# ShengkaiWu/IoU-aware-single-stage-object-detector

Hardware: AMD Instinct MI355X
Metric: images/sec at 1333x800, IoU-aware RetinaNet R-50-FPN (higher is better)
Workload: dtype fp32; 1 GPU; IoU-aware RetinaNet R-50-FPN fp32, batch 8 per GPU, 3x800x1344 (1333x800 padded to /32), random-init weights, whole inference path incl. NMS, device-to-host copy and bbox2result (the reference's simple_test: per-class arrays on the host; batch i's host part runs under batch i+1's device part, the last one inside the timed region); global_batch=8, parallelism=dp1, dets_per_image=100

## Files before the change

### include/iouaware.h

```cpp
#ifndef IOUAWARE_H
#define IOUAWARE_H

#include <stddef.h>
#include <stdint.h>

#ifdef __cplusplus
extern "C" {
#endif

#define IA_MAX_LEVELS 8
#define IA_MAX_ANCHORS 16
#define IA_MAX_NMS_PRE 4096
#define IA_MAX_CANDIDATES 8192
#define IA_MAX_PER_IMG 1024

#define IA_F32 0
#define IA_BF16 1
#define IA_F16 2
#define IA_F64 3

#define IA_LAYOUT_NCHW 0
#define IA_LAYOUT_NHWC 1

#define IA_CLS_SIGMOID 0
// ... 124 lines not shown
    int32_t dst_channels, dst_offset;
    float *dst[IA_MAX_LEVELS];
} ia_wino_seg;
int ia_wino_tiles(const ia_wino_geom *g, int32_t *tiles);
int ia_wino_input_transform(const ia_wino_geom *g, const float *const *x, int channels, int groups,
                            const float *pre_scale, const float *pre_shift, int pre_relu, float *V,
                            void *stream);
int ia_wino_output_transform(const ia_wino_geom *g, const float *M, int channels, int groups,
                             const float *bias, int relu, int nseg, const ia_wino_seg *segs,
                             void *stream);
int ia_wino_mid_transform(const ia_wino_geom *g, const float *M, int channels, int groups_m,
                          const float *bias, int relu, float *V, int groups_v, void *stream);
int ia_wino_in_gemm(const ia_wino_geom *g, const float *const *x, int channels, const float *pre_scale,
                    const float *pre_shift, int pre_relu, const float *u_packed, float *M, void *stream);

int ia_wino_grad_output_transform(const ia_wino_geom *g, const float *const *dy, int channels,
                                  float *dM, void *stream);

#define IA_COLSUM_MAX_STRIPS 512
size_t ia_relu_bwd_bias_grad_workspace_bytes(int64_t rows, int n);
int ia_wino_weight_transform(const float *w, int n_in, int n_out, int64_t stride_in,
                             int64_t stride_out, int64_t stride_ky, int64_t stride_kx, int flip,
                             const double *G, float *U, void *stream);
int ia_wino_weight_grad(const float *dU, int n_in, int n_out, const double *G, float *dW,
                        int64_t stride_in, int64_t stride_out, int64_t stride_ky, int64_t stride_kx,
                        void *stream);
int ia_bn_fold_fwd(const float *w, const float *gamma, const float *beta, const float *mean,
                   const float *inv_std, int cout, int K, float *w_out, float *b_out, void *stream);
int ia_bn_fold_bwd(const float *dw_folded, const float *db_folded, const float *w, const float *gamma,
                   const float *mean, const float *inv_std, int cout, int K, float *dw,
                   float *dgamma, float *dbeta, void *stream);
int ia_relu_bwd_bias_grad(const float *dy, const float *y, int64_t rows, int n, float *g, float *db,
                          void *workspace, size_t workspace_bytes, void *stream);

int ia_linear_bias_act(const float *A, const float *W, const float *bias, const float *residual,
                       float *D, int64_t rows, int k, int n, int relu, void *workspace,
                       size_t workspace_bytes, void *stream);
int ia_linear_bias_act_bf16(const void *A, const void *W, const float *bias, const void *residual,
                            void *D, int64_t rows, int k, int n, int relu, void *workspace,
                            size_t workspace_bytes, void *stream);
int ia_batched_gemm(const float *A, const float *W, float *D, int batch, int64_t rows, int k, int n,
                    void *workspace, size_t workspace_bytes, void *stream);
int ia_batched_gemm_stream(const float *A, const float *W, float *D, int batch, int64_t rows, int k,
                           int n, void *stream);

size_t ia_im2col3x3_bytes(int B, int H, int W, int C, int stride, int dtype);
int ia_im2col3x3_nhwc(const void *x, void *col, int B, int H, int W, int C, int stride, int dtype,
                      void *stream);
int ia_conv1x1_strided(const void *x, const void *W_kn, const float *bias, const void *residual,
                       void *D, int B, int H, int W, int k, int n, int stride, int relu, int dtype,
                       void *workspace, size_t workspace_bytes, void *stream);
int ia_col2im3x3_nhwc(const void *dcol, void *dx, int B, int H, int W, int C, int stride, int dtype,
                      void *stream);

size_t ia_deform_im2col3x3_bytes(int B, int H, int W, int C, int stride, int pad, int dil);
int ia_deform_im2col3x3_nhwc(const float *x, const float *offset, int64_t offset_pix_stride,
                             const float *mask, int64_t mask_pix_stride, int mask_logits,
                             float *col, int B, int H, int W, int C, int stride, int pad,
                             int dil, int deformable_groups, void *stream);
int ia_deform_col2im3x3_nhwc(const float *dcol, const float *x, const float *offset,
                             int64_t offset_pix_stride, const float *mask,
                             int64_t mask_pix_stride, float *dx, float *d_offset, float *d_mask,
                             int B, int H, int W, int C, int stride, int pad, int dil,
                             int deformable_groups, void *stream);

int ia_gemm_tuning(int mode);

int ia_gemm_table_add(int64_t m, int64_t n, int64_t k, int flags, int batch, int dtype,
                      int solution_index);
int ia_gemm_table_clear(void);
int ia_gemm_table_dump(int64_t *rows7, int capacity);
int ia_gemm_table_stats(int64_t *hits_misses_stale);
int ia_gemm_library_version(void);

int ia_linear_bias_act_wt(const float *A, const float *W_nk, const float *bias,
                          const float *residual, float *D, int64_t rows, int k, int n, int relu,
                          void *workspace, size_t workspace_bytes, void *stream);
int ia_gemm_tn(const float *G, const float *X, float *D, int batch, int64_t rows, int n, int k,
               void *workspace, size_t workspace_bytes, void *stream);


int ia_focal_loss_fwd(const void *cls, int dtype, const int64_t *labels,
                      const float *label_weights, int B, int A, int C, int HW, float gamma,
                      float alpha, double *loss_sum, void *stream);
int ia_focal_loss_bwd(const void *cls, int dtype, const int64_t *labels,
                      const float *label_weights, int B, int A, int C, int HW, float gamma,
                      float alpha, float gscale, const float *gscale_dev, float *grad_cls,
                      void *stream);

int ia_smooth_l1_fwd(const void *pred, int dtype, const float *target, const float *weight,
                     int B, int A, int HW, float beta, double *loss_sum, void *stream);
int ia_smooth_l1_bwd(const void *pred, int dtype, const float *target, const float *weight,
                     int B, int A, int HW, float beta, float gscale, const float *gscale_dev,
                     float *grad_pred, void *stream);

int ia_balanced_l1_fwd(const void *pred, int dtype, const float *target, const float *weight,
                       int B, int A, int HW, float beta, float alpha, float gamma, double *loss_sum,
                       void *stream);
int ia_balanced_l1_bwd(const void *pred, int dtype, const float *target, const float *weight,
                       int B, int A, int HW, float beta, float alpha, float gamma, float gscale,
                       const float *gscale_dev, float *grad_pred, void *stream);

int ia_focal_loss_balanced_fwd(const void *cls, int dtype, const int64_t *labels,
                               const float *label_weights, const float *anchor_iou, int B, int A,
                               int C, int HW, float gamma, float alpha, float eta,
                               double *loss_sums3, void *stream);
// ... 345 lines not shown
```

### iou-aware-single-stage-object-detector_amd/csrc/build.py

```python
import os
import subprocess
import sys

HERE = os.path.dirname(os.path.abspath(__file__))
SOURCES = ['capi.hip', 'decode.hip', 'select.hip', 'nms.hip', 'loss.hip', 'elementwise.hip', 'assign.hip',
           'softnms.hip', 'preproc.hip', 'wino.hip', 'gemm.hip', 'lazynms.hip', 'headloss.hip', 'gconv.hip',
           'trainops.hip', 'bignms.hip', 'conv3x3_bf16.hip', 'conv3x3_bf16_bwd.hip', 'conv1x1_stream.hip', 'im2col.hip', 'nms64.hip', 'stem.hip',
           'groupnorm.hip', 'pointdecode.hip', 'pointloss.hip', 'gconv_bf16.hip', 'gconv_bwd.hip', 'deform.hip']
HEADERS = ['ia_math.hpp', 'ia_block.hpp', 'ia_internal.hpp', 'ia_loss.hpp', 'ia_headloss.hpp', 'ia_rowmax_dev.hpp', 'ia_gather_dev.hpp', 'ia_nms.hpp', 'ia_conv3.hpp', 'ia_wino.hpp', '../../include/iouaware.h']
OUT = os.path.join(HERE, 'libiouaware_hip.so')
FLAGS = ['--offload-arch=gfx950', '-O3', '-std=c++17', '-fPIC', '-ffp-contract=off',
         '-fhip-fp32-correctly-rounded-divide-sqrt', '-fno-gpu-rdc',
         '-Wall', '-Wno-unused-function']


def _hipcc():
    for c in (os.environ.get('HIPCC'), '/opt/rocm/bin/hipcc', 'hipcc'):
        if c and (os.path.isabs(c) and os.path.exists(c) or not os.path.isabs(c)):
            return c
    return 'hipcc'


def needs_build():
    if not os.path.exists(OUT):
        return True
    t = os.path.getmtime(OUT)
    deps = [os.path.join(HERE, f) for f in SOURCES + HEADERS] + [os.path.abspath(__file__)]
    return any(os.path.getmtime(d) > t for d in deps)


def build(force=False, verbose=False):
    if not force and not needs_build():
        return OUT
    objs = []
    procs = []
    for src in SOURCES:
        obj = os.path.join(HERE, src.replace('.hip', '.o'))
        cmd = [_hipcc()] + FLAGS + ['-c', os.path.join(HERE, src), '-o', obj]
        if verbose:
            print(' '.join(cmd))
        procs.append((src, subprocess.Popen(cmd, stdout=subprocess.PIPE, stderr=subprocess.STDOUT)))
        objs.append(obj)
    for src, pr in procs:
        out, _ = pr.communicate()
        if pr.returncode != 0:
            raise RuntimeError('hipcc failed on %s:\n%s' % (src, out.decode()))
        if verbose and out:
            print(out.decode())
    cmd = [_hipcc(), '--offload-arch=gfx950', '-shared', '-fPIC', '-o', OUT] + objs + [
        '-L/opt/rocm/lib', '-lhipblaslt', '-Wl,-rpath,/opt/rocm/lib']
    subprocess.run(cmd, check=True)
    return OUT


if __name__ == '__main__':
    print(build(force='--force' in sys.argv, verbose=True))
```

### iou-aware-single-stage-object-detector_amd/iouaware/_lib.py

```python
import ctypes as C
import os

IA_MAX_LEVELS = 8
IA_MAX_ANCHORS = 16
IA_MAX_NMS_PRE = 4096
IA_MAX_CANDIDATES = 8192
IA_MAX_PER_IMG = 1024
IA_F32, IA_BF16, IA_F16, IA_F64 = 0, 1, 2, 3
IA_LAYOUT_NCHW, IA_LAYOUT_NHWC = 0, 1
IA_CLS_SIGMOID, IA_CLS_SOFTMAX = 0, 1
IA_CLS_SIGMOID_NOIOU, IA_CLS_SOFTMAX_NOIOU = 2, 3
IA_LOSS_SLOTS = 64
IA_MAX_TARGET_BATCH = 16
IA_GN_CHUNK = 256

_CSRC = os.path.join(os.path.dirname(os.path.abspath(__file__)), '..', 'csrc')
SO_PATH = os.path.abspath(os.path.join(_CSRC, 'libiouaware_hip.so'))


class HeadGeom(C.Structure):
    _fields_ = [('num_levels', C.c_int32), ('num_anchors', C.c_int32),
                ('num_classes', C.c_int32), ('nms_pre', C.c_int32),
                ('H', C.c_int32 * IA_MAX_LEVELS), ('W', C.c_int32 * IA_MAX_LEVELS),
                ('stride', C.c_int32 * IA_MAX_LEVELS),
# ... 170 lines not shown
    'ia_focal_loss_balanced_fwd': (_i, [_vp, _i, _vp, _vp, _vp, _i, _i, _i, _i, _f, _f, _f, _vp, _vp]),
    'ia_focal_loss_balanced_bwd': (_i, [_vp, _i, _vp, _vp, _vp, _i, _i, _i, _i, _f, _f, _f, _vp, _f,
                                        _vp, _vp, _vp]),
    'ia_smooth_l1_balanced_fwd': (_i, [_vp, _i, _vp, _vp, _vp, _i, _i, _i, _f, _f, _vp, _vp]),
    'ia_smooth_l1_balanced_bwd': (_i, [_vp, _i, _vp, _vp, _vp, _i, _i, _i, _f, _f, _f, _vp, _vp,
                                       _vp]),
    'ia_iou_bce_fwd': (_i, [_G, _i, _vp, _vp, _i, _vp, _vp, _i, _vp, _vp, _vp]),
    'ia_iou_bce_bwd': (_i, [_G, _i, _vp, _vp, _i, _vp, _vp, _i, _f, _vp, _vp, _vp, _vp]),
    'ia_anchor_targets': (_i, [_G, _vp, _vp, _vp, _i, _i, _vp, _f, _f, _f, _f, _vp, _vp, _vp, _vp,
                               _vp, _vp, _vp]),
    'ia_anchor_targets_ptrs': (_i, [_G, C.POINTER(C.c_void_p), C.POINTER(C.c_void_p),
                                    C.POINTER(C.c_int32), _i, C.POINTER(C.c_int32), _f, _f, _f, _f,
                                    _vp, _vp, _vp, _vp, _vp, _vp, _vp]),
    'ia_head_loss_workspace_bytes': (_sz, [_G, _i]),
    'ia_head_loss_workspace_bytes_cfg': (_sz, [_G, _i, C.POINTER(HeadLossCfg)]),
    'ia_head_loss_fwd': (_i, [_G, _P, _i, _i, C.POINTER(HeadTargets), C.POINTER(HeadLossCfg), _vp,
                              _sz, _vp, _vp]),
    'ia_head_loss_bwd': (_i, [_G, _P, _i, _i, C.POINTER(HeadTargets), C.POINTER(HeadLossCfg), _vp,
                              _vp, _vp, _P, _vp]),
    'ia_head_loss_fwd_nhwc': (_i, [_G, _P, C.POINTER(LevelPixStrides), _i, C.POINTER(HeadTargets),
                                   C.POINTER(HeadLossCfg), _vp, _sz, _vp, _vp]),
    'ia_head_loss_bwd_nhwc': (_i, [_G, _P, C.POINTER(LevelPixStrides), _i, C.POINTER(HeadTargets),
                                   C.POINTER(HeadLossCfg), _vp, _vp, _P, C.POINTER(LevelPixStrides),
                                   _vp]),
    'ia_head_loss_fwd_box': (_i, [_G, _P, _i, _i, C.POINTER(HeadTargets), C.POINTER(HeadLossCfg),
                                  C.POINTER(BoxLossCfg), _vp, _sz, _vp, _vp]),
    'ia_head_loss_bwd_box': (_i, [_G, _P, _i, _i, C.POINTER(HeadTargets), C.POINTER(HeadLossCfg),
                                  C.POINTER(BoxLossCfg), _vp, _vp, _vp, _P, _vp]),
    'ia_head_loss_fwd_nhwc_box': (_i, [_G, _P, C.POINTER(LevelPixStrides), _i, C.POINTER(HeadTargets),
                                       C.POINTER(HeadLossCfg), C.POINTER(BoxLossCfg), _vp, _sz, _vp, _vp]),
    'ia_head_loss_bwd_nhwc_box': (_i, [_G, _P, C.POINTER(LevelPixStrides), _i, C.POINTER(HeadTargets),
                                       C.POINTER(HeadLossCfg), C.POINTER(BoxLossCfg), _vp, _vp, _P,
                                       C.POINTER(LevelPixStrides), _vp]),
    'ia_grouped_conv3x3_pack': (_i, [_vp, _vp, _i, _i, _vp]),
    'ia_grouped_conv3x3_nhwc': (_i, [_vp, _vp, _vp, _vp, _i, _i, _i, _i, _i, _i, _i, _vp]),
    'ia_grouped_conv3x3_packed_bytes_bf16': (C.c_size_t, [_i, _i]),
    'ia_grouped_conv3x3_pack_dev': (_i, [_vp, _vp, _i, _i, _i, _vp, _vp]),
    'ia_grouped_conv3x3_bwd_data_nhwc': (_i, [_vp, _vp, _vp, _i, _i, _i, _i, _i, _i, _vp]),
    'ia_grouped_conv3x3_bwd_weight_workspace_bytes': (C.c_size_t, [_i, _i, _i, _i, _i, _i]),
    'ia_grouped_conv3x3_bwd_weight_nhwc': (_i, [_vp, _vp, _vp, _vp, C.c_size_t, _i, _i, _i, _i, _i, _i, _vp]),
    'ia_grouped_conv3x3_pack_bf16': (_i, [_vp, _vp, _i, _i, _vp]),
    'ia_grouped_conv3x3_bf16_nhwc': (_i, [_vp, _vp, _vp, _vp, _i, _i, _i, _i, _i, _i, _i, _vp]),
    'ia_sigmoid_focal_loss_fwd': (_i, [_vp, _vp, _i, _i, _f, _f, _vp, _vp]),
    'ia_sigmoid_focal_loss_bwd': (_i, [_vp, _vp, _vp, _i, _i, _f, _f, _vp, _vp]),
    'ia_sigmoid_focal_loss_fwd_dt': (_i, [_vp, _i, _vp, _i, _i, _f, _f, _vp, _vp]),
    'ia_sigmoid_focal_loss_bwd_dt': (_i, [_vp, _i, _vp, _vp, _i, _i, _f, _f, _vp, _vp]),
    'ia_channel_affine_act': (_i, [_vp, _i, _vp, _vp, _vp, _vp, _vp, _i, _i, _i, _i64, _vp]),
    'ia_channel_affine_act_nhwc': (_i, [_vp, _i, _vp, _vp, _vp, _vp, _vp, _i, _i64, _i, _vp]),
    'ia_nhwc_to_nchw': (_i, [_vp, _vp, _i, _i, _i, _i64, _vp]),
    'ia_upsample2x_add_nhwc': (_i, [_vp, _vp, _i, _i, _i, _i, _i, _i, _vp]),
    'ia_conv1x1_stream': (_i, [_vp, _vp, _vp, _vp, _vp, C.c_int64, _i, _i, _i, _vp]),
    'ia_stem_conv7x7s2': (_i, [_vp, _vp, _vp, _i, _i, _i, _vp]),
    'ia_stem_conv7x7s2_bf16': (_i, [_vp, _vp, _vp, _i, _i, _i, _vp]),
    'ia_conv1x1_wide': (_i, [_vp, _vp, _vp, _vp, _vp, C.c_int64, _i, _i, _i, _vp]),
    'ia_conv1x1_chain': (_i, [_vp, _vp, _vp, _vp, _vp, _vp, _vp, _vp, _i64, _i, _i, _i, _vp]),
    'ia_conv3x3_bf16_packed_bytes': (C.c_size_t, [_i, _i, _i]),
    'ia_conv3x3_bf16_pack': (_i, [_vp, _i, _i, _i, _vp, _vp]),
    'ia_conv3x3_bf16_levels': (_i, [_vp, _vp, _vp, _i, _vp]),
    'ia_conv3x3_bf16_wgrad_workspace_bytes': (C.c_size_t, [_vp]),
    'ia_conv3x3_bf16_wgrad_plan': (_i, [_vp, C.POINTER(C.c_int32), C.POINTER(C.c_int32), C.POINTER(C.c_int32)]),
    'ia_conv3x3_bf16_wgrad_levels': (_i, [_vp, _vp, _vp, C.c_size_t, _vp]),
    'ia_conv3x3_bf16_pack_f32': (_i, [_vp, _i, _i, _i, _i, _vp, _vp]),
    'ia_relu_bwd_bias_grad_bf16_workspace_bytes': (C.c_size_t, [C.c_int64, _i]),
    'ia_relu_bwd_bias_grad_bf16': (_i, [_vp, C.c_int64, _vp, C.c_int64, C.c_int64, _i, _vp, C.c_int64, _vp,
                                        _vp, C.c_size_t, _vp]),
    'ia_upsample2x_add_nhwc_dt': (_i, [_vp, _vp, _i, _i, _i, _i, _i, _i, _i, _vp]),
    'ia_affine_relu_maxpool_nhwc_dt': (_i, [_vp, _i, _vp, _vp, _i, _i, _i, _i, _vp, _vp]),
    'ia_affine_relu_maxpool_nhwc': (_i, [_vp, _vp, _vp, _i, _i, _i, _i, _vp, _vp]),
    'ia_groupnorm_workspace_bytes': (_sz, [_WG, _i, _i]),
    'ia_groupnorm_stats': (_i, [_WG, C.POINTER(C.c_void_p), _i, _i, _vp, _sz, _vp]),
    'ia_groupnorm_apply': (_i, [_WG, C.POINTER(C.c_void_p), _i, _i, _vp, _vp, _f, _i, _vp, _sz, _vp]),
    'ia_groupnorm_workspace_bytes_dt': (_sz, [_WG, _i, _i, _i]),
    'ia_groupnorm_stats_dt': (_i, [_WG, C.POINTER(C.c_void_p), _i, _i, _i, _vp, _sz, _vp]),
    'ia_groupnorm_apply_dt': (_i, [_WG, C.POINTER(C.c_void_p), _i, _i, _i, _vp, _vp, _f, _i, _vp, _sz,
                                   _vp]),
    'ia_groupnorm_saved_bytes': (_sz, [_WG, _i, _i]),
    'ia_groupnorm_apply_to': (_i, [_WG, C.POINTER(C.c_void_p), C.POINTER(C.c_void_p), _i, _i, _vp, _vp, _f,
                                   _i, _vp, _sz, _vp, _sz, _vp]),
    'ia_groupnorm_bwd_workspace_bytes': (_sz, [_WG, _i, _i]),
    'ia_groupnorm_bwd_reduce': (_i, [_WG, C.POINTER(C.c_void_p), C.POINTER(C.c_void_p), _i, _i, _vp, _vp, _i,
                                     _vp, _sz, _vp, _sz, _vp]),
    'ia_groupnorm_bwd_apply': (_i, [_WG, C.POINTER(C.c_void_p), C.POINTER(C.c_void_p),
                                    C.POINTER(C.c_void_p), _i, _i, _vp, _vp, _i, _vp, _sz, _vp, _sz, _vp,
                                    _vp, _vp]),
    'ia_groupnorm_saved_bytes_dt': (_sz, [_WG, _i, _i, _i]),
    'ia_groupnorm_apply_to_dt': (_i, [_WG, C.POINTER(C.c_void_p), C.POINTER(C.c_void_p), _i, _i, _i, _vp, _vp,
                                      _f, _i, _vp, _sz, _vp, _sz, _vp]),
    'ia_groupnorm_bwd_workspace_bytes_dt': (_sz, [_WG, _i, _i, _i]),
    'ia_groupnorm_bwd_reduce_dt': (_i, [_WG, C.POINTER(C.c_void_p), C.POINTER(C.c_void_p), _i, _i, _i, _vp, _vp,
                                        _i, _vp, _sz, _vp, _sz, _vp]),
    'ia_groupnorm_bwd_apply_dt': (_i, [_WG, C.POINTER(C.c_void_p), C.POINTER(C.c_void_p),
                                       C.POINTER(C.c_void_p), _i, _i, _i, _vp, _vp, _i, _vp, _sz, _vp, _sz,
                                       _vp, _vp, _vp]),
    'ia_scale_exp_levels': (_i, [_WG, C.POINTER(C.c_void_p), _i, _vp, _vp]),
    'ia_scale_exp_levels_dt': (_i, [_WG, C.POINTER(C.c_void_p), _i, _i, _vp, _vp]),
    'ia_point_workspace_bytes': (_sz, [_PG, _i]),
    'ia_point_workspace_layout': (_i, [_PG, _i, C.POINTER(_sz * 8)]),
    'ia_point_decode_stage': (_i, [_PG, _P, _i, _vp, _vp, _i, _vp, _sz, _vp]),
    'ia_point_get_bboxes': (_i, [_PG, _P, _i, _vp, _vp, _i, _f, _f, _i, _i, _vp, _sz, _vp, _vp, _vp,
                                 _vp, _vp]),
    'ia_point_ctr_decode_stage': (_i, [_PG, _P, _i, _vp, _vp, _i, _f, _vp, _sz, _vp]),
    'ia_point_ctr_get_bboxes': (_i, [_PG, _P, _i, _vp, _vp, _i, _f, _f, _i, _i, _vp, _sz, _vp, _vp,
                                     _vp, _vp, _vp]),
    'ia_point_decode_stage_dt': (_i, [_PG, _P, _i, _i, _vp, _vp, _i, _vp, _sz, _vp]),
    'ia_point_get_bboxes_dt': (_i, [_PG, _P, _i, _i, _vp, _vp, _i, _f, _f, _i, _i, _vp, _sz, _vp, _vp,
                                    _vp, _vp, _vp]),
    'ia_point_ctr_decode_stage_dt': (_i, [_PG, _P, _i, _i, _vp, _vp, _i, _f, _vp, _sz, _vp]),
# ... 50 lines not shown
```

### iou-aware-single-stage-object-detector_amd/iouaware/fuse.py

```python
import types

import torch
import torch.nn.functional as F
from torch.nn.modules.batchnorm import _BatchNorm

from . import ops, train_fuse
from .backbones import BasicBlock, Bottleneck, ResNet
from .deform_conv import _DeformBase, _one
from .layers import ConvModule, Scale
from .winograd import plain_3x3

_VEC = {torch.float32: 4, torch.bfloat16: 8}


def _fold_bn(bn):
    if not isinstance(bn, _BatchNorm):
        raise TypeError('only BatchNorm can be folded, got %s' % type(bn).__name__)
    with torch.no_grad():
        var, mean = bn.running_var.float(), bn.running_mean.float()
        g = bn.weight.float() if bn.weight is not None else torch.ones_like(var)
        b = bn.bias.float() if bn.bias is not None else torch.zeros_like(var)
        scale = g / torch.sqrt(var + bn.eps)
        shift = b - mean * scale
    return scale.contiguous(), shift.contiguous()
# ... 92 lines not shown
        om = co(out).contiguous(memory_format=torch.channels_last)
    n = 18 * self.deformable_groups
    return ops.deform_conv3x3(out, om[:, :n], om[:, n:] if self.with_modulated_dcn else None, f['dcn2'],
                              f['b2'], _one(c2.stride, 'stride'), _one(c2.padding, 'padding'),
                              _one(c2.dilation, 'dilation'), self.deformable_groups, relu=True,
                              mask_logits=True)


def _bottleneck_run(self, x, h1=None, nxt=None):
    if not _fast(self, x):
        if _train(self) and train_fuse.bottleneck_usable(self, x):
            return train_fuse.bottleneck_forward(self, x), None
        return type(self).forward(self, x), None
    f = self._ia_fused
    lt = 'w1' in f and x.dtype in (torch.float32, torch.bfloat16) \
        and x.is_contiguous(memory_format=torch.channels_last)
    if h1 is not None:
        w, out, pre = f, h1, None
    elif lt:
        w = _weights_for(f, x.dtype)
        out, pre = ops.linear_bias_act(x, w['w1'], f['b1'], relu=True), None
    else:
        out, pre = self.conv1(x), (f['s1'], f['b1'], True)
    gw = f.get('gconv2')
    wino = f.get('wino2')
    if getattr(self, 'with_dcn', False):
        if pre is not None:
            out = ops.channel_affine_act_(out, f['s1'], f['b1'], relu=True)
        out = _dcn_conv2(self, f, out)
    elif gw is not None and out.dtype == torch.float32 \
            and out.is_contiguous(memory_format=torch.channels_last):
        if pre is not None:
            out = ops.channel_affine_act_(out, f['s1'], f['b1'], relu=True)
        out = ops.grouped_conv3x3(out, gw, f['b2'], self.conv2.groups, self.conv2.stride[0],
                                  relu=True)
    elif gw is not None and out.dtype == torch.bfloat16 and self.conv2.in_channels % 32 == 0 \
            and out.is_contiguous(memory_format=torch.channels_last) and self._ia_gconv_bf16:
        if pre is not None:
            out = ops.channel_affine_act_(out, f['s1'], f['b1'], relu=True)
        wp = f.get('_gconv2_bf16')
        if wp is None:
            wp = f['_gconv2_bf16'] = ops.pack_grouped_weight_bf16(self.conv2.weight, f['s2'])
        out = ops.grouped_conv3x3_bf16(out, wp, f['b2'], self.conv2.groups, self.conv2.stride[0],
                                       relu=True)
    elif wino is not None and wino.usable(out):
        out = wino(out, pre=pre)
    elif pre is None and 'c3' in f and out.dtype == torch.bfloat16 \
            and out.is_contiguous(memory_format=torch.channels_last):
        wp = f.get('_c3_packed')
        if wp is None:
            wp = f['_c3_packed'] = ops.conv3x3_bf16_pack(f['c3'])
        out = ops.conv3x3_bf16(out, wp, f['b2'], self.conv2.out_channels, relu=True)
    elif lt and 'im2col2' in f and out.is_contiguous(memory_format=torch.channels_last):
        out = ops.conv3x3_im2col(out, w['im2col2'], f['b2'], stride=self.conv2.stride[0], relu=True)
    else:
        if pre is not None:
            out = ops.channel_affine_act_(out, f['s1'], f['b1'], relu=True)
        out = ops.channel_affine_act_(self.conv2(out), f['s2'], f['b2'], relu=True)
    if lt and out.is_contiguous(memory_format=torch.channels_last):
        if self.downsample is None:
            if nxt is not None:
                return ops.conv1x1_chain(out, w['w3'], f['b3'], x, nxt['w1'], nxt['b1'])
            return ops.linear_bias_act(out, w['w3'], f['b3'], residual=x, relu=True), None
        if 'wd' in f:
            idn = ops.linear_bias_act(x, w['wd'], f['b3d'])
            if nxt is not None:
                return ops.conv1x1_chain(out, w['w3'], None, idn, nxt['w1'], nxt['b1'])
            return ops.linear_bias_act(out, w['w3'], None, residual=idn, relu=True), None
        ds = self.downsample[0]
        if 'wd_s' in f:
            idn = ops.conv1x1_strided(x, w['wd_s'], None, None, stride=ds.stride[0])
        else:
            idn = F.conv2d(x, w['wd_conv'], None, ds.stride, ds.padding)
        return ops.linear_bias_act(out, w['w3'], f['b3d'], residual=idn, relu=True), None
    out = self.conv3(out)
    if self.downsample is None:
        return ops.channel_affine_act_(out, f['s3'], f['b3'], residual=x, relu=True), None
    idn = self.downsample[0](x)
    return ops.channel_affine_act_(out, f['s3'], f['b3'], residual=idn, res_scale=f['sd'],
                                   res_shift=f['bd'], relu=True), None


def _chain_ok(blk, nxt, x):
    f, g = getattr(blk, '_ia_fused', None), getattr(nxt, '_ia_fused', None)
    if f is None or g is None or 'w3' not in f or 'w1' not in g or nxt.downsample is not None:
        return False
    if getattr(blk, 'with_dcn', False) or getattr(nxt, 'with_dcn', False):
        return False
    if blk.downsample is not None and 'wd' not in f:
        return False
    k, n = f['w3'].shape
    return tuple(g['w1'].shape) == (n, g['w1'].shape[1]) and ops.chain_usable(x, k, n, g['w1'].shape[1]) \
        and x.is_contiguous(memory_format=torch.channels_last)


def _has_hooks(m):
    import torch.nn.modules.module as tm
    return bool(m._forward_hooks or m._forward_pre_hooks or tm._global_forward_hooks
                or tm._global_forward_pre_hooks)


def _layer_forward(self, x):
    blocks = list(self)
    if not all(isinstance(b, Bottleneck) and hasattr(b, '_ia_opts') for b in blocks) or not blocks:
        return torch.nn.Sequential.forward(self, x)
    h1 = None
    for i, blk in enumerate(blocks):
# ... 421 lines not shown
```

### iou-aware-single-stage-object-detector_amd/iouaware/ops.py

```python
import ctypes as C
import os

import numpy as np
import torch

from . import _lib
from ._lib import HeadGeom, LevelPtrs, IA_F32, IA_BF16


_raw_stream = getattr(torch._C, '_cuda_getCurrentRawStream', None)


def stream_id():
    if _raw_stream is not None:
        return _raw_stream(torch.cuda.current_device())
    return torch.cuda.current_stream().cuda_stream


def _stream():
    return C.c_void_p(stream_id())


def _ptr(t):
    return C.c_void_p(t.data_ptr()) if t is not None else C.c_void_p(0)
# ... 897 lines not shown
    B, Cc, H, W = x.shape
    if x.dtype != torch.float32 or not x.is_contiguous(memory_format=torch.channels_last):
        raise TypeError('im2col3x3 needs a channels-last fp32 activation')
    stride = int(stride)
    if Cc % 4 or not 1 <= stride <= 4:
        raise ValueError('im2col3x3: C a multiple of 4, stride 1..4')
    rows = B * ((H - 1) // stride + 1) * ((W - 1) // stride + 1)
    nbytes = rows * 9 * Cc * 4
    col = _col_buffer(x.device, nbytes)
    _lib.check(_lib.lib().ia_im2col3x3_nhwc(_ptr(x), _ptr(col), B, H, W, Cc, stride, IA_F32, _stream()),
               'ia_im2col3x3_nhwc')
    return col[:nbytes].view(torch.float32).view(rows, 9 * Cc)


def conv3x3_dcol(g, w_kn):
    _require_gpu(g, 'g')
    B, n, Ho, Wo = g.shape
    if g.dtype != torch.float32 or not g.is_contiguous(memory_format=torch.channels_last):
        raise TypeError('conv3x3_dcol needs a channels-last fp32 gradient')
    if w_kn.dim() != 2 or w_kn.shape[1] != n or w_kn.shape[0] % 9 or not w_kn.is_contiguous() \
            or w_kn.dtype != torch.float32:
        raise ValueError('weight must be the contiguous fp32 (9 * C, Cout) matrix of the forward')
    rows, k9 = B * Ho * Wo, int(w_kn.shape[0])
    nbytes = rows * k9 * 4
    col = _col_buffer(g.device, nbytes)
    _ensure_gemm_table()
    ws = _workspace(g.device, _LT_WS_BYTES)
    _lib.check(_lib.lib().ia_linear_bias_act_wt(_ptr(g), _ptr(w_kn), None, None, _ptr(col), rows, n, k9, 0,
                                                _ptr(ws), _LT_WS_BYTES, _stream()),
               'ia_linear_bias_act_wt (dcol)')
    return col[:nbytes].view(torch.float32).view(rows, k9)


def col2im3x3(dcol, B, H, W, C, stride):
    _require_gpu(dcol, 'dcol')
    B, H, W, C, stride = int(B), int(H), int(W), int(C), int(stride)
    if not 1 <= stride <= 4 or min(B, H, W, C) < 1 or C % 4:
        raise ValueError('col2im3x3: stride 1..4, positive sizes, C a multiple of 4')
    rows = B * ((H - 1) // stride + 1) * ((W - 1) // stride + 1)
    if dcol.dtype != torch.float32 or not dcol.is_contiguous() or dcol.numel() != rows * 9 * C:
        raise ValueError('col2im3x3: dcol must be a contiguous fp32 (B * Ho * Wo, 9 * C) matrix')
    dx = torch.empty((B, C, H, W), dtype=torch.float32, device=dcol.device,
                     memory_format=torch.channels_last)
    _lib.check(_lib.lib().ia_col2im3x3_nhwc(_ptr(dcol), _ptr(dx), B, H, W, C, stride, IA_F32, _stream()),
               'ia_col2im3x3_nhwc')
    return dx


def conv3x3_weight_kn(weight, scale=None):
    w = weight.detach().float()
    if scale is not None:
        w = w * scale.view(-1, 1, 1, 1)
    return w.permute(2, 3, 1, 0).reshape(9 * w.shape[1], w.shape[0]).contiguous()


DEFORM_COL_CAP = 256 << 20


def deform_out_hw(H, W, stride, padding, dilation):
    e = 2 * int(dilation) + 1
    return (H + 2 * padding - e) // stride + 1, (W + 2 * padding - e) // stride + 1


def _rows_ps(t, what, B, ch, Ho, Wo):
    if t.dtype != torch.float32:
        raise TypeError('%s must be float32, got %s' % (what, t.dtype))
    if tuple(t.shape) != (B, ch, Ho, Wo):
        raise ValueError('%s must have shape %s, got %s' % (what, (B, ch, Ho, Wo), tuple(t.shape)))
    ps = t.stride(3) if Wo > 1 else (t.stride(2) if Ho > 1 else (t.stride(0) if B > 1 else ch))
    if t.stride(1) != 1 or ps < ch or (Ho > 1 and Wo > 1 and t.stride(2) != Wo * ps) \
            or (B > 1 and t.stride(0) != Ho * Wo * ps):
        raise ValueError('%s must be channels-last (or a channel slice of a channels-last tensor)' % what)
    return int(ps)


def _deform_check(x, offset, mask, stride, padding, dilation, dg):
    _require_gpu(x, 'x')
    _require_gpu(offset, 'offset')
    if x.dtype != torch.float32:
        raise TypeError('the deformable convolution kernels are fp32, got %s' % x.dtype)
    if x.dim() != 4 or not x.is_contiguous(memory_format=torch.channels_last):
        raise ValueError('x must be a channels-last (B, C, H, W) tensor')
    stride, padding, dilation, dg = int(stride), int(padding), int(dilation), int(dg)
    if stride < 1 or padding < 0 or dilation < 1 or dg < 1:
        raise ValueError('stride / dilation / deformable_groups >= 1, padding >= 0')
    B, Cc, H, W = (int(v) for v in x.shape)
    if Cc % (4 * dg):
        raise ValueError('deformable_groups: C = %d must be a multiple of 4 * deformable_groups = %d'
                         % (Cc, 4 * dg))
    Ho, Wo = deform_out_hw(H, W, stride, padding, dilation)
    if Ho < 1 or Wo < 1:
        raise ValueError('the %d x %d map is smaller than the dilated kernel' % (H, W))
    ops_ = _rows_ps(offset, 'offset', B, dg * 18, Ho, Wo)
    mps = 0
    if mask is not None:
        _require_gpu(mask, 'mask')
        mps = _rows_ps(mask, 'mask', B, dg * 9, Ho, Wo)
    return B, Cc, H, W, Ho, Wo, ops_, mps, (stride, padding, dilation, dg)


def deform_im2col3x3(x, offset, mask=None, stride=1, padding=1, dilation=1, deformable_groups=1,
                     mask_logits=False, out=None):
    B, Cc, H, W, Ho, Wo, ops_, mps, (s, p, d, dg) = _deform_check(x, offset, mask, stride, padding,
                                                                 dilation, deformable_groups)
    rows = B * Ho * Wo
    nbytes = rows * 9 * Cc * 4
# ... 1021 lines not shown
```

Before: 413.6 img/s.

## Add implicit-GEMM fp32 MFMA kernel for stride-2 3x3 conv in layer2

```diff
diff --git a/include/iouaware.h b/include/iouaware.h
--- a/include/iouaware.h
+++ b/include/iouaware.h
@@ -200,6 +200,10 @@
                        void *workspace, size_t workspace_bytes, void *stream);
 int ia_col2im3x3_nhwc(const void *dcol, void *dx, int B, int H, int W, int C, int stride, int dtype,
                       void *stream);
+int64_t ia_conv3x3_s2_packed_floats(int cin, int cout);
+int ia_conv3x3_s2_pack(const float *w_kn, int cin, int cout, float *packed, void *stream);
+int ia_conv3x3_s2_f32(const float *x, const float *packed, const float *bias, float *y, int B, int H,
+                      int W, int cin, int cout, int stride, int relu, int block, void *stream);
 
 size_t ia_deform_im2col3x3_bytes(int B, int H, int W, int C, int stride, int pad, int dil);
 int ia_deform_im2col3x3_nhwc(const float *x, const float *offset, int64_t offset_pix_stride,
diff --git a/iou-aware-single-stage-object-detector_amd/csrc/build.py b/iou-aware-single-stage-object-detector_amd/csrc/build.py
--- a/iou-aware-single-stage-object-detector_amd/csrc/build.py
+++ b/iou-aware-single-stage-object-detector_amd/csrc/build.py
@@ -6,7 +6,8 @@
 SOURCES = ['capi.hip', 'decode.hip', 'select.hip', 'nms.hip', 'loss.hip', 'elementwise.hip', 'assign.hip',
            'softnms.hip', 'preproc.hip', 'wino.hip', 'gemm.hip', 'lazynms.hip', 'headloss.hip', 'gconv.hip',
            'trainops.hip', 'bignms.hip', 'conv3x3_bf16.hip', 'conv3x3_bf16_bwd.hip', 'conv1x1_stream.hip', 'im2col.hip', 'nms64.hip', 'stem.hip',
-           'groupnorm.hip', 'pointdecode.hip', 'pointloss.hip', 'gconv_bf16.hip', 'gconv_bwd.hip', 'deform.hip']
+           'groupnorm.hip', 'pointdecode.hip', 'pointloss.hip', 'gconv_bf16.hip', 'gconv_bwd.hip', 'deform.hip',
+           'conv3x3_s2.hip']
 HEADERS = ['ia_math.hpp', 'ia_block.hpp', 'ia_internal.hpp', 'ia_loss.hpp', 'ia_headloss.hpp', 'ia_rowmax_dev.hpp', 'ia_gather_dev.hpp', 'ia_nms.hpp', 'ia_conv3.hpp', 'ia_wino.hpp', '../../include/iouaware.h']
 OUT = os.path.join(HERE, 'libiouaware_hip.so')
 FLAGS = ['--offload-arch=gfx950', '-O3', '-std=c++17', '-fPIC', '-ffp-contract=off',
diff --git a/iou-aware-single-stage-object-detector_amd/csrc/conv3x3_s2.hip b/iou-aware-single-stage-object-detector_amd/csrc/conv3x3_s2.hip
--- /dev/null
+++ b/iou-aware-single-stage-object-detector_amd/csrc/conv3x3_s2.hip
@@ -0,0 +1,267 @@
+#include "ia_internal.hpp"
+
+namespace ia {
+
+typedef float f32x2 __attribute__((ext_vector_type(2)));
+typedef float f32x4 __attribute__((ext_vector_type(4)));
+
+constexpr int S2_TN = 128;
+constexpr int S2_KC = 32;
+constexpr int S2_QU = 2 * 4 * S2_TN * 4;
+
+struct S2Args {
+    const float *x;
+    const float *wp;
+    const float *bias;
+    float *y;
+    int32_t H, W, Ho, Wo, Cin, Cout, P, n_nb, n_pb, relu;
+};
+
+__device__ __host__ __forceinline__ int s2_swz(int row, int q, int g) { return row ^ (((q ^ g) & 3) << 1); }
+
+template <int PX>
+__global__ void __launch_bounds__(256, PX == 128 ? 2 : 3) k_conv3x3_s2(S2Args a)
+{
+    constexpr int WN = PX % 32 == 0 ? 2 : 1, WM = 4 / WN;
+    constexpr int NI = S2_TN / 16 / WM, NJ = PX / 16 / WN;
+    constexpr int NIT = (PX + 31) / 32;
+    constexpr int QV = 2 * 4 * PX * 4;
+    constexpr int SLOTS = 8 * NI * NJ, HALF = SLOTS / 2;
+    static_assert(PX % 16 == 0 && NIT + 4 <= HALF && 2 * NIT + 4 <= HALF, "block shape");
+    __shared__ __attribute__((aligned(16))) float lds[2 * (QV + S2_QU)];
+    const int tid = threadIdx.x, lane = tid & 63;
+    const int wave = __builtin_amdgcn_readfirstlane(tid >> 6);
+    const int xcd = blockIdx.x & 7, r = blockIdx.x >> 3;
+    const int nb = r % a.n_nb, pb = (r / a.n_nb) * 8 + xcd;
+    if (pb >= a.n_pb) return;
+    const int ncs = a.Cin / S2_KC, nst = 9 * ncs;
+    const int wm = wave % WM, wn = wave / WM;
+
+    const int j8 = tid & 7, vr = tid >> 3;
+    const int vg = j8 >> 2, vj4 = j8 & 3;
+    const float *xc[NIT];
+    int vm[NIT], vw[NIT][2];
+    const bool act_last = PX % 32 == 0 || vr + 32 * (NIT - 1) < PX;
+#pragma unroll
+    for (int it = 0; it < NIT; ++it) {
+        const int row = (it == NIT - 1 && !act_last) ? vr : vr + 32 * it;
+        int gp = pb * PX + row;
+        const bool live = gp < a.P;
+        gp = live ? gp : a.P - 1;
+        const int b = gp / (a.Ho * a.Wo), rem = gp - b * (a.Ho * a.Wo);
+        const int yo = rem / a.Wo, xo = rem - yo * a.Wo;
+        xc[it] = a.x + (((size_t)b * a.H + 2 * yo) * a.W + 2 * xo) * a.Cin + 4 * j8;
+        int m = 0;
+#pragma unroll
+        for (int tap = 0; tap < 9; ++tap) {
+            const int yi = 2 * yo + tap / 3 - 1, xi = 2 * xo + tap % 3 - 1;
+            if (live && yi >= 0 && yi < a.H && xi >= 0 && xi < a.W) m |= 1 << tap;
+        }
+        vm[it] = m;
+#pragma unroll
+        for (int h = 0; h < 2; ++h) {
+            const int q = 2 * (vj4 & 1) + h;
+            vw[it][h] = ((vg * 4 + q) * PX + s2_swz(row, q, vg)) * 4 + 2 * (vj4 >> 1);
+        }
+    }
+    const float *usrc = a.wp + ((size_t)nb * nst) * S2_QU + tid * 4;
+
+    const int q = lane >> 4, t = lane & 15;
+    int ru[2], rv[2];
+#pragma unroll
+    for (int g = 0; g < 2; ++g) {
+        ru[g] = ((g * 4 + q) * S2_TN + 16 * NI * wm + s2_swz(t, q, g)) * 4;
+        rv[g] = ((g * 4 + q) * PX + 16 * NJ * wn + s2_swz(t, q, g)) * 4;
+    }
+    f32x4 acc[NI][NJ];
+#pragma unroll
+    for (int i = 0; i < NI; ++i)
+#pragma unroll
+        for (int j = 0; j < NJ; ++j) acc[i][j] = f32x4{0.f, 0.f, 0.f, 0.f};
+
+#define S2_PIN() __builtin_amdgcn_sched_barrier(0)
+    f32x4 sv[2][NIT], su[2][4];
+    int stap[2];
+    auto request = [&](int set, int stage) {
+        const int tap = stage / ncs, cs = stage - tap * ncs;
+        const int toff = ((tap / 3 - 1) * a.W + (tap % 3 - 1)) * a.Cin;
+        stap[set] = tap;
+#pragma unroll
+        for (int it = 0; it < NIT; ++it)
+            if (it < NIT - 1 || act_last) sv[set][it] = *reinterpret_cast<const f32x4 *>(xc[it] + cs * S2_KC + (((vm[it] >> tap) & 1) ? toff : 0));
+#pragma unroll
+        for (int it = 0; it < 4; ++it)
+            su[set][it] = *reinterpret_cast<const f32x4 *>(usrc + (size_t)stage * S2_QU + it * 1024);
+    };
+    request(0, 0);
+    request(1, nst > 1 ? 1 : 0);
+    {
+        float *lv = lds, *lu = lds + QV;
+#pragma unroll
+        for (int it = 0; it < NIT; ++it) {
+            if (it == NIT - 1 && !act_last) continue;
+            const f32x4 v = ((vm[it] >> stap[0]) & 1) ? sv[0][it] : f32x4{0.f, 0.f, 0.f, 0.f};
+#pragma unroll
+            for (int h = 0; h < 2; ++h)
+                *reinterpret_cast<f32x2 *>(lv + vw[it][h]) = f32x2{v[2 * h], v[2 * h + 1]};
+        }
+#pragma unroll
+        for (int it = 0; it < 4; ++it) *reinterpret_cast<f32x4 *>(lu + tid * 4 + it * 1024) = su[0][it];
+    }
+    __syncthreads();
+
+    for (int s2 = 0; s2 < nst; s2 += 2) {
+#pragma unroll
+        for (int par = 0; par < 2; ++par) {
+            const int s = s2 + par;
+            if (s >= nst) break;
+            const float *lv = lds + par * (QV + S2_QU), *lu = lv + QV;
+            float *wv = lds + (par ^ 1) * (QV + S2_QU), *wu = wv + QV;
+            const int sn = (s + 2 < nst) ? s + 2 : nst - 1;
+            const int ntap = sn / ncs, ncs_i = sn - ntap * ncs;
+            const int ntoff = ((ntap / 3 - 1) * a.W + (ntap % 3 - 1)) * a.Cin;
+            const int otap = stap[par ^ 1];
+#pragma unroll
+            for (int g = 0; g < 2; ++g) {
+                f32x4 fu[NI], fv[NJ];
+#pragma unroll
+                for (int i = 0; i < NI; ++i) fu[i] = *reinterpret_cast<const f32x4 *>(lu + ru[g] + i * 64);
+#pragma unroll
+                for (int j = 0; j < NJ; ++j) fv[j] = *reinterpret_cast<const f32x4 *>(lv + rv[g] + j * 64);
+                S2_PIN();
+#pragma unroll
+                for (int ks = 0; ks < 4; ++ks) {
+#pragma unroll
+                    for (int i = 0; i < NI; ++i)
+#pragma unroll
+                        for (int j = 0; j < NJ; ++j) {
+                            acc[i][j] = __builtin_amdgcn_mfma_f32_16x16x4f32(fu[i][ks], fv[j][ks], acc[i][j], 0, 0, 0);
+                            S2_PIN();
+                            const int slot = ((g * 4 + ks) * NI + i) * NJ + j;
+                            if (slot >= HALF && slot < HALF + 2 * NIT) {
+                                const int it = (slot - HALF) >> 1, h = (slot - HALF) & 1;
+                                const bool in = (vm[it] >> otap) & 1;
+                                if (it < NIT - 1 || act_last) *reinterpret_cast<f32x2 *>(wv + vw[it][h]) =
+                                    f32x2{in ? sv[par ^ 1][it][2 * h] : 0.f, in ? sv[par ^ 1][it][2 * h + 1] : 0.f};
+                            } else if (slot >= HALF + 2 * NIT && slot < HALF + 2 * NIT + 4) {
+                                const int it = slot - HALF - 2 * NIT;
+                                *reinterpret_cast<f32x4 *>(wu + tid * 4 + it * 1024) = su[par ^ 1][it];
+                            }
+                            if (slot < NIT) {
+                                if (slot < NIT - 1 || act_last) sv[par][slot] = *reinterpret_cast<const f32x4 *>(
+                                    xc[slot] + ncs_i * S2_KC + (((vm[slot] >> ntap) & 1) ? ntoff : 0));
+                            } else if (slot < NIT + 4) {
+                                su[par][slot - NIT] = *reinterpret_cast<const f32x4 *>(usrc + (size_t)sn * S2_QU + (slot - NIT) * 1024);
+                            }
+                            S2_PIN();
+                        }
+                }
+            }
+            stap[par] = ntap;
+            __syncthreads();
+        }
+    }
+#undef S2_PIN
+    const int c0 = nb * S2_TN + 16 * NI * wm + 4 * q;
+    if (c0 >= a.Cout) return;
+    f32x4 bv[NI];
+#pragma unroll
+    for (int i = 0; i < NI; ++i)
+        bv[i] = a.bias ? *reinterpret_cast<const f32x4 *>(a.bias + c0 + 16 * i) : f32x4{0.f, 0.f, 0.f, 0.f};
+#pragma unroll
+    for (int j = 0; j < NJ; ++j) {
+        const int gp = pb * PX + 16 * NJ * wn + 16 * j + t;
+        if (gp >= a.P) continue;
+        float *dst = a.y + (size_t)gp * a.Cout + c0;
+#pragma unroll
+        for (int i = 0; i < NI; ++i) {
+            f32x4 v = acc[i][j] + bv[i];
+            if (a.relu) {
+#pragma unroll
+                for (int e = 0; e < 4; ++e) v[e] = v[e] < 0.f ? 0.f : v[e];
+            }
+            *reinterpret_cast<f32x4 *>(dst + 16 * i) = v;
+        }
+    }
+}
+
+__global__ void k_conv3x3_s2_pack(const float *w, float *out, int K, int N, int64_t total)
+{
+    const int64_t idx = (int64_t)blockIdx.x * blockDim.x + threadIdx.x;
+    if (idx >= total) return;
+    const int j = (int)(idx & 3);
+    const int cp = (int)((idx >> 2) & 127), q = (int)((idx >> 9) & 3), g = (int)((idx >> 11) & 1);
+    const int64_t rest = idx >> 12;
+    const int nst = K / S2_KC;
+    const int s = (int)(rest % nst), nb = (int)(rest / nst);
+    const int cout = s2_swz(cp, q, g);
+    const int k = 32 * s + 16 * g + 8 * (j >> 1) + 2 * q + (j & 1), n = nb * S2_TN + cout;
+    out[idx] = (n < N) ? w[(size_t)k * N + n] : 0.0f;
+}
+
+static int pick_block(int64_t pixels, int n_nb)
+{
+    static int cus = 0;
+    if (cus <= 0) {
+        int dev = 0, n = 0;
+        if (hipGetDevice(&dev) != hipSuccess ||
+            hipDeviceGetAttribute(&n, hipDeviceAttributeMultiprocessorCount, dev) != hipSuccess || n < 1)
+            n = 256;
+        cus = n;
+    }
+    int best = 128;
+    int64_t t_best = 0;
+    for (int px : {128, 64, 48}) {
+        const int64_t wgs = (pixels + px - 1) / px * n_nb, t = (wgs + cus - 1) / cus * px;
+        if (px == 128 || t < t_best) { best = px; t_best = t; }
+    }
+    return best;
+}
+
+}
+
+extern "C" {
+
+int64_t ia_conv3x3_s2_packed_floats(int cin, int cout)
+{
+    if (cin < ia::S2_KC || (cin % ia::S2_KC) || cout < 64 || (cout % 64)) return IA_E_ARG;
+    const int64_t n_nb = (cout + ia::S2_TN - 1) / ia::S2_TN;
+    return n_nb * (9 * cin / ia::S2_KC) * ia::S2_QU;
+}
+
+int ia_conv3x3_s2_pack(const float *w_kn, int cin, int cout, float *packed, void *stream)
+{
+    const int64_t total = ia_conv3x3_s2_packed_floats(cin, cout);
+    if (!w_kn || !packed || total < 0 || (((uintptr_t)w_kn | (uintptr_t)packed) & 15)) return IA_E_ARG;
+    hipLaunchKernelGGL(ia::k_conv3x3_s2_pack, dim3((unsigned)((total + 255) / 256)), dim3(256), 0,
+                       (hipStream_t)stream, w_kn, packed, 9 * cin, cout, total);
+    return ia::hip_status(hipGetLastError());
+}
+
+int ia_conv3x3_s2_f32(const float *x, const float *packed, const float *bias, float *y, int B, int H,
+                      int W, int cin, int cout, int stride, int relu, int block, void *stream)
+{
+    if (!x || !packed || !y || B < 1 || H < 1 || W < 1 || stride != 2) return IA_E_ARG;
+    if (cin < ia::S2_KC || (cin % ia::S2_KC) || cout < 64 || (cout % 64)) return IA_E_ARG;
+    if (block != 0 && block != 48 && block != 64 && block != 128) return IA_E_ARG;
+    if (((uintptr_t)x | (uintptr_t)packed | (uintptr_t)y | (uintptr_t)bias) & 15) return IA_E_ARG;
+    const int Ho = (H - 1) / 2 + 1, Wo = (W - 1) / 2 + 1;
+    const int64_t pixels = (int64_t)B * Ho * Wo;
+    if (pixels > 2147483647LL - 128 || 2LL * W * cin > 2147483647LL) return IA_E_ARG;
+    ia::S2Args a;
+    a.x = x; a.wp = packed; a.bias = bias; a.y = y;
+    a.H = H; a.W = W; a.Ho = Ho; a.Wo = Wo; a.Cin = cin; a.Cout = cout; a.P = (int32_t)pixels;
+    a.n_nb = (cout + ia::S2_TN - 1) / ia::S2_TN; a.relu = relu ? 1 : 0;
+    const int px = block ? block : ia::pick_block(pixels, a.n_nb);
+    a.n_pb = (int32_t)((pixels + px - 1) / px);
+    const int64_t wgs = ((int64_t)a.n_pb + 7) / 8 * 8 * a.n_nb;
+    if (wgs > 2147483647LL) return IA_E_ARG;
+    const dim3 grid((unsigned)wgs);
+    hipStream_t s = (hipStream_t)stream;
+    if (px == 48) hipLaunchKernelGGL(ia::k_conv3x3_s2<48>, grid, dim3(256), 0, s, a);
+    else if (px == 64) hipLaunchKernelGGL(ia::k_conv3x3_s2<64>, grid, dim3(256), 0, s, a);
+    else hipLaunchKernelGGL(ia::k_conv3x3_s2<128>, grid, dim3(256), 0, s, a);
+    return ia::hip_status(hipGetLastError());
+}
+
+}
diff --git a/iou-aware-single-stage-object-detector_amd/iouaware/_lib.py b/iou-aware-single-stage-object-detector_amd/iouaware/_lib.py
--- a/iou-aware-single-stage-object-detector_amd/iouaware/_lib.py
+++ b/iou-aware-single-stage-object-detector_amd/iouaware/_lib.py
@@ -246,7 +246,10 @@
     'ia_conv1x1_stream': (_i, [_vp, _vp, _vp, _vp, _vp, C.c_int64, _i, _i, _i, _vp]),
     'ia_stem_conv7x7s2': (_i, [_vp, _vp, _vp, _i, _i, _i, _vp]),
     'ia_stem_conv7x7s2_bf16': (_i, [_vp, _vp, _vp, _i, _i, _i, _vp]),
-    'ia_conv1x1_wide': (_i, [_vp, _vp, _vp, _vp, _vp, C.c_int64, _i, _i, _i, _vp]),
+    'ia_conv3x3_s2_packed_floats': (C.c_int64, [_i, _i]),
+    'ia_conv3x3_s2_pack': (_i, [_vp, _i, _i, _vp, _vp]),
+    'ia_conv3x3_s2_f32': (_i, [_vp, _vp, _vp, _vp, _i, _i, _i, _i, _i, _i, _i, _i, _vp]),
+    'ia_conv1x1_wide':(_i, [_vp, _vp, _vp, _vp, _vp, C.c_int64, _i, _i, _i, _vp]),
     'ia_conv1x1_chain': (_i, [_vp, _vp, _vp, _vp, _vp, _vp, _vp, _vp, _i64, _i, _i, _i, _vp]),
     'ia_conv3x3_bf16_packed_bytes': (C.c_size_t, [_i, _i, _i]),
     'ia_conv3x3_bf16_pack': (_i, [_vp, _i, _i, _i, _vp, _vp]),
diff --git a/iou-aware-single-stage-object-detector_amd/iouaware/fuse.py b/iou-aware-single-stage-object-detector_amd/iouaware/fuse.py
--- a/iou-aware-single-stage-object-detector_amd/iouaware/fuse.py
+++ b/iou-aware-single-stage-object-detector_amd/iouaware/fuse.py
@@ -168,7 +168,13 @@
             wp = f['_c3_packed'] = ops.conv3x3_bf16_pack(f['c3'])
         out = ops.conv3x3_bf16(out, wp, f['b2'], self.conv2.out_channels, relu=True)
     elif lt and 'im2col2' in f and out.is_contiguous(memory_format=torch.channels_last):
-        out = ops.conv3x3_im2col(out, w['im2col2'], f['b2'], stride=self.conv2.stride[0], relu=True)
+        if ops.conv3x3_s2_usable(out, self.conv2.in_channels, self.conv2.out_channels, self.conv2.stride[0]):
+            wp = f.get('_s2_packed')
+            if wp is None:
+                wp = f['_s2_packed'] = ops.conv3x3_s2_pack(f['im2col2'])
+            out = ops.conv3x3_s2(out, wp, f['b2'], self.conv2.out_channels, relu=True)
+        else:
+            out = ops.conv3x3_im2col(out, w['im2col2'], f['b2'], stride=self.conv2.stride[0], relu=True)
     else:
         if pre is not None:
             out = ops.channel_affine_act_(out, f['s1'], f['b1'], relu=True)
diff --git a/iou-aware-single-stage-object-detector_amd/iouaware/ops.py b/iou-aware-single-stage-object-detector_amd/iouaware/ops.py
--- a/iou-aware-single-stage-object-detector_amd/iouaware/ops.py
+++ b/iou-aware-single-stage-object-detector_amd/iouaware/ops.py
@@ -973,6 +973,57 @@
     if scale is not None:
         w = w * scale.view(-1, 1, 1, 1)
     return w.permute(2, 3, 1, 0).reshape(9 * w.shape[1], w.shape[0]).contiguous()
+
+
+S2_IMPLICIT = True
+_S2_ROUTED = ((128, 128, 32768),)
+
+
+def conv3x3_s2_usable(x, cin, cout, stride=2):
+    if not S2_IMPLICIT or stride != 2 or x.dtype != torch.float32 or x.dim() != 4 or x.shape[1] != cin \
+            or not x.is_cuda or not x.is_contiguous(memory_format=torch.channels_last):
+        return False
+    pixels = x.shape[0] * ((x.shape[2] - 1) // 2 + 1) * ((x.shape[3] - 1) // 2 + 1)
+    return any((cin, cout) == (ci, co) and pixels >= p for ci, co, p in _S2_ROUTED)
+
+
+def conv3x3_s2_pack(w_kn):
+    _require_gpu(w_kn, 'w_kn')
+    if w_kn.dim() != 2 or w_kn.dtype != torch.float32 or not w_kn.is_contiguous() or w_kn.shape[0] % 9:
+        raise ValueError('conv3x3_s2_pack: a contiguous fp32 (9 * Cin, Cout) matrix')
+    cin, cout = int(w_kn.shape[0]) // 9, int(w_kn.shape[1])
+    L = _lib.lib()
+    n = L.ia_conv3x3_s2_packed_floats(cin, cout)
+    if n < 0:
+        raise ValueError('conv3x3_s2_pack: Cin must be a multiple of 32 and Cout a multiple of 64')
+    packed = torch.empty(int(n), dtype=torch.float32, device=w_kn.device)
+    _lib.check(L.ia_conv3x3_s2_pack(_ptr(w_kn), cin, cout, _ptr(packed), _stream()), 'ia_conv3x3_s2_pack')
+    return packed
+
+
+def conv3x3_s2(x, packed, bias, cout, relu=False, stride=2, block=0):
+    _require_gpu(x, 'x')
+    if x.dim() != 4 or x.dtype != torch.float32 or not x.is_contiguous(memory_format=torch.channels_last):
+        raise TypeError('conv3x3_s2 needs a channels-last fp32 activation')
+    if int(stride) != 2:
+        raise ValueError('conv3x3_s2: stride 2 only')
+    B, Cc, H, W = x.shape
+    cout = int(cout)
+    L = _lib.lib()
+    n = L.ia_conv3x3_s2_packed_floats(Cc, cout)
+    if n < 0:
+        raise ValueError('conv3x3_s2: Cin must be a multiple of 32 and Cout a multiple of 64')
+    if packed.dtype != torch.float32 or packed.numel() != n or not packed.is_contiguous() \
+            or packed.device != x.device:
+        raise ValueError('conv3x3_s2: packed must be conv3x3_s2_pack of the (9 * Cin, Cout) weight')
+    if bias is not None and (bias.dtype != torch.float32 or bias.numel() != cout or not bias.is_contiguous()
+                             or bias.device != x.device):
+        raise TypeError('conv3x3_s2: bias must be a contiguous fp32 vector of Cout values')
+    Ho, Wo = (H - 1) // 2 + 1, (W - 1) // 2 + 1
+    out = torch.empty((B, cout, Ho, Wo), dtype=torch.float32, device=x.device, memory_format=torch.channels_last)
+    _lib.check(L.ia_conv3x3_s2_f32(_ptr(x), _ptr(packed), _ptr(bias), _ptr(out), B, H, W, Cc, cout, 2,
+                                   int(bool(relu)), int(block), _stream()), 'ia_conv3x3_s2_f32')
+    return out
 
 
 DEFORM_COL_CAP = 256 << 20
```

Measured after the change: 414.6 img/s (median of 6 runs). No clear change (+0.2%).
